# gio54321/quill-zkvm

Hardware: AMD Instinct MI355X
Metric: G1 MSM scalars/sec at 2^24 + sumcheck-prover ms at 2^20 vars (1/8 GPU) (higher is better)
Workload: dtype u256-montgomery (BN254 Fr scalars, Fq coordinates); 1 GPU; KZG commit / Pippenger G1 MSM, 2^24 BN254 scalars per GPU; parallelism=msm-shard-by-base-index x1

## Files before the change

### quill-zkvm_amd/csrc/msm.hip

```cpp
#include <stdlib.h>
#include <string.h>

#include "common.h"
#include "curve29.h"

using namespace qg;

namespace qg {

static constexpr int MSM_BLOCK = 256;

static int msm_window_bits(size_t n) {
  int best = 4;
  double best_cost = 1e300;
  for (int c = 4; c <= 22; c++) {
    const int W = (255 + c - 1) / c;
    const int k = 254 - c * (W - 1);
    if (k < 30 && (n >> k) > 4096) continue;
    const double cost = (double)n * W + 12.0 * (double)((size_t)1 << (c - 1));
    if (cost < best_cost) {
      best_cost = cost;
      best = c;
    }
  }
  return best;
}

QG_DEV Fr fr_canon29(const Fr& x) {
  F29<FrP> k = F29<FrP>::zero();
  k.l[0] = 32;
  return from29(canon29(mul29(to29(x), k)));
}

template <class Emit>
QG_DEV void for_each_digit(const Fr& canon, int c, int W, Emit&& emit) {
  uint32_t v[8];
#pragma unroll
  for (int i = 0; i < 8; i++) v[i] = canon.v[i];
  const uint32_t mask = (1u << c) - 1u;
  const uint32_t half = 1u << (c - 1);
  const uint32_t full = 1u << c;
  uint32_t carry = 0;
  for (int w = 0; w < W; w++) {
    const uint32_t d = (v[0] & mask) + carry;
    if (d > half) {
      carry = 1;
      const uint32_t mag = full - d;
      if (mag) emit(w, mag - 1, true);
    } else {
      carry = 0;
      if (d) emit(w, d - 1, false);
    }
#pragma unroll
    for (int i = 0; i < 7; i++) v[i] = __builtin_amdgcn_alignbit(v[i + 1], v[i], (uint32_t)c);
    v[7] >>= c;
  }
}

QG_DEV uint32_t xcd_tile(uint32_t b, uint32_t G) {
  const uint32_t x = b & 7u, q = G >> 3, r = G & 7u;
  return x * q + (x < r ? x : r) + (b >> 3);
}

static constexpr int SORT_BLOCK = 256;
static constexpr int SORT_TILE_MAX = 1024;
static constexpr size_t SORT_LDS_A = 72 * 1024;
static constexpr int SORT_CHUNK = 8192;
static constexpr int SORT_H_MAX = 1024, SORT_NL_MAX = 4096;

__global__ void k_handover_tag(uint32_t* hv, uint32_t w, uint32_t gen, uint32_t clear) {
  if (threadIdx.x == 0) {
    if (clear) hv[1] = hv[2] = hv[3] = 0u;
    hv[w] = gen;
  }
}

QG_DEV void msm_handover_check(uint32_t* hv, uint32_t w0, uint32_t nw, uint32_t gen, uint32_t bit) {
  if (hv == nullptr || threadIdx.x != 0) return;
  for (uint32_t w = w0; w < w0 + nw; w++)
    if (__hip_atomic_load(hv + w, __ATOMIC_RELAXED, __HIP_MEMORY_SCOPE_AGENT) != gen) {
      atomicOr(hv + 1, bit);
      return;
    }
}

__global__ void __launch_bounds__(SORT_BLOCK)
    k_sortA_hist(const Fr* __restrict__ scalars, size_t n, int c, int W, int LO, int H,
                 uint32_t nblk, uint32_t tile, uint32_t* __restrict__ hrow, Fr* __restrict__ canon,
                 uint32_t* hv, uint32_t gen, int wsel, int canon_ready) {
  extern __shared__ uint32_t hist[];
  msm_handover_check(hv, 0, 1, gen, 1u);
  for (int g = threadIdx.x; g < H; g += blockDim.x) hist[g] = 0;
  __syncthreads();
  const uint32_t tb = xcd_tile(blockIdx.x, nblk);
  const size_t base = (size_t)tb * tile;
  const size_t end = base + tile < n ? base + tile : n;
  for (size_t i = base + threadIdx.x; i < end; i += blockDim.x) {
    Fr s;
    if (canon_ready) {
      s = canon[i];
    } else {
      s = fr_canon29(scalars[i]);
      canon[i] = s;
    }
    for_each_digit(s, c, W, [&](int w, uint32_t b, bool) {
      if (wsel < 0 || w == wsel) atomicAdd(&hist[b >> LO], 1u);
    });
  }
  __syncthreads();
  for (int g = threadIdx.x; g < H; g += blockDim.x) hrow[(size_t)tb * H + g] = hist[g];
}

__global__ void __launch_bounds__(256)
    k_transpose32(const uint32_t* __restrict__ in, uint32_t rows, uint32_t cols,
                  uint32_t* __restrict__ out) {
  __shared__ uint32_t tile[32][33];
  const uint32_t c0 = blockIdx.x * 32, r0 = blockIdx.y * 32;
  const uint32_t tx = threadIdx.x & 31, ty = threadIdx.x >> 5;
  for (uint32_t k = ty; k < 32; k += 8)
    if (r0 + k < rows && c0 + tx < cols) tile[k][tx] = in[(size_t)(r0 + k) * cols + c0 + tx];
  __syncthreads();
  for (uint32_t k = ty; k < 32; k += 8)
    if (c0 + k < cols && r0 + tx < rows) out[(size_t)(c0 + k) * rows + r0 + tx] = tile[tx][k];
}

template <int BLK>
__device__ void lds_exscan(uint32_t* a, int n, uint32_t* tmp ) {
  const int per = (n + BLK - 1) / BLK;
  const int b = threadIdx.x * per;
  const int lane = threadIdx.x & 63, wid = threadIdx.x >> 6;
  uint32_t tot = 0;
  for (int k = 0; k < per; k++)
    if (b + k < n) tot += a[b + k];
  uint32_t inc = tot;
#pragma unroll
  for (int d = 1; d < 64; d <<= 1) {
    const uint32_t y = __shfl_up(inc, d, 64);
    if (lane >= d) inc += y;
  }
  if (lane == 63) tmp[wid] = inc;
  __syncthreads();
  uint32_t run = inc - tot;
  for (int w = 0; w < wid; w++) run += tmp[w];
  for (int k = 0; k < per; k++) {
    if (b + k < n) {
      const uint32_t v = a[b + k];
      a[b + k] = run;
      run += v;
    }
  }
  __syncthreads();
}

__device__ __forceinline__ int lds_upper(const uint32_t* off, int n, uint32_t p) {
  int lo = 0, hi = n;
  while (hi - lo > 1) {
    int mid = (lo + hi) >> 1;
    if (off[mid] <= p) lo = mid;
    else hi = mid;
  }
  return lo;
}

template <int BLK>
__global__ void __launch_bounds__(BLK)
    k_sortA_scatter(const Fr* __restrict__ canon, size_t n, size_t N, size_t off, int c, int W, int LO,
                    int H,
                    uint32_t nblk, uint32_t tile, const uint32_t* __restrict__ hrow,
                    const uint32_t* __restrict__ orow, uint32_t* __restrict__ tmp_e,
                    uint16_t* __restrict__ tmp_l, int wsel) {
  extern __shared__ __attribute__((aligned(16))) unsigned char smem[];
  uint32_t* ent = reinterpret_cast<uint32_t*>(smem);
  uint32_t* bkt = ent + (size_t)tile * (wsel < 0 ? W : 1);
  uint32_t* loff = bkt + (size_t)tile * (wsel < 0 ? W : 1);
  uint32_t* cur = loff + H;
  uint32_t* gb = cur + H;
  uint32_t* scr = gb + H;
  (void)scr;
  const uint32_t tb = xcd_tile(blockIdx.x, nblk);
  const size_t base = (size_t)tb * tile;
  const size_t end = base + tile < n ? base + tile : n;
  static_assert(SORT_TILE_MAX % BLK == 0, "pass-A tile must split evenly over the block");
  constexpr int PER = SORT_TILE_MAX / BLK;
  Fr sv[PER];
#pragma unroll
  for (int j = 0; j < PER; j++) {
    const size_t i = base + threadIdx.x + (size_t)j * BLK;
    if (i < end) sv[j] = canon[i];
  }
  for (int g = threadIdx.x; g < H; g += blockDim.x) {
    loff[g] = hrow[(size_t)tb * H + g];
    gb[g] = orow[(size_t)tb * H + g];
    cur[g] = 0;
  }
  __syncthreads();
#pragma unroll
  for (int j = 0; j < PER; j++) {
    const size_t i = base + threadIdx.x + (size_t)j * BLK;
    if (i >= end) break;
    for_each_digit(sv[j], c, W, [&](int w, uint32_t b, bool neg) {
      if (wsel >= 0 && w != wsel) return;
      const uint32_t g = b >> LO;
      const uint32_t slot = loff[g] + atomicAdd(&cur[g], 1u);
      const size_t row = (wsel < 0 ? (size_t)w * N : 0) + off + i;
      ent[slot] = (uint32_t)row | (neg ? 0x80000000u : 0u);
      bkt[slot] = b;
    });
  }
  __syncthreads();
  const uint32_t total = loff[H - 1] + cur[H - 1];
  const uint32_t lmask = (1u << LO) - 1u;
  for (uint32_t p = threadIdx.x; p < total; p += blockDim.x) {
    const uint32_t b = bkt[p];
    const uint32_t dst = gb[b >> LO] + p;
    tmp_e[dst] = ent[p];
    tmp_l[dst] = (uint16_t)(b & lmask);
  }
}

template <int BLK>
__global__ void __launch_bounds__(BLK)
    k_sortA_rows(uint32_t* __restrict__ hrow, uint32_t* __restrict__ orow, int H) {
  __shared__ uint32_t a[SORT_H_MAX], scr[BLK / 64];
  const size_t r = (size_t)blockIdx.x * H;
  for (int g = threadIdx.x; g < H; g += blockDim.x) a[g] = hrow[r + g];
  __syncthreads();
  lds_exscan<BLK>(a, H, scr);
  for (int g = threadIdx.x; g < H; g += blockDim.x) {
    hrow[r + g] = a[g];
    orow[r + g] -= a[g];
  }
}

__global__ void __launch_bounds__(1024)
    k_sort_chunks(const uint32_t* __restrict__ goff, uint32_t nblk, int H, uint32_t chunk,
                  uint32_t* __restrict__ gstart, uint32_t* __restrict__ cbase,
                  uint32_t* __restrict__ chunk_group, uint32_t* __restrict__ misc) {
  __shared__ uint32_t sh[1024];
  const int g = threadIdx.x;
  if (threadIdx.x >= 1 && threadIdx.x <= 3) misc[threadIdx.x] = threadIdx.x == 2 ? 0xffffffffu : 0u;
  const uint32_t total = goff[(size_t)H * nblk];
  uint32_t gs = 0, ge = 0, nch = 0;
  if (g < H) {
    gs = goff[(size_t)g * nblk];
    ge = (g + 1 < H) ? goff[(size_t)(g + 1) * nblk] : total;
    nch = (ge - gs + chunk - 1) / chunk;
    gstart[g] = gs;
  }
  sh[threadIdx.x] = nch;
  __syncthreads();
  for (int off = 1; off < 1024; off <<= 1) {
    uint32_t add = threadIdx.x >= (unsigned)off ? sh[threadIdx.x - off] : 0u;
    __syncthreads();
    sh[threadIdx.x] += add;
    __syncthreads();
  }
  const uint32_t cb = sh[threadIdx.x] - nch;
  if (g < H) {
    cbase[g] = cb;
    for (uint32_t k = 0; k < nch; k++) chunk_group[cb + k] = (uint32_t)g;
  }
  if (threadIdx.x == 1023) {
    gstart[H] = total;
    cbase[H] = sh[1023];
    misc[0] = sh[1023];
  }
}

template <int BLK, int CHUNK>
__global__ void __launch_bounds__(BLK)
    k_sortB_hist(const uint16_t* __restrict__ tmp_l, const uint32_t* __restrict__ gstart,
                 const uint32_t* __restrict__ cbase, const uint32_t* __restrict__ chunk_group,
                 const uint32_t* __restrict__ nchunks, int NL, uint32_t* __restrict__ chist) {
  extern __shared__ uint32_t hist[];
  const uint32_t nch = *nchunks;
  if (blockIdx.x >= nch) return;
  const uint32_t k = xcd_tile(blockIdx.x, nch);
  const uint32_t g = chunk_group[k];
  const uint32_t s = gstart[g] + (k - cbase[g]) * CHUNK;
  const uint32_t e = min(s + CHUNK, gstart[g + 1]);
  for (int l = threadIdx.x; l < NL; l += blockDim.x) hist[l] = 0;
  __syncthreads();
  constexpr int PER = CHUNK / BLK;
  uint32_t lv[PER];
#pragma unroll
  for (int j = 0; j < PER; j++) {
    const uint32_t p = s + threadIdx.x + j * BLK;
    lv[j] = p < e ? (uint32_t)tmp_l[p] : 0xffffffffu;
  }
#pragma unroll
  for (int j = 0; j < PER; j++)
    if (lv[j] != 0xffffffffu) atomicAdd(&hist[lv[j]], 1u);
  __syncthreads();
  for (int l = threadIdx.x; l < NL; l += blockDim.x) chist[(size_t)k * NL + l] = hist[l];
}

__global__ void k_sort_bucket_count(const uint32_t* __restrict__ cbase, const uint32_t* __restrict__ chist,
                                    int LO, uint32_t nb, uint32_t* __restrict__ counts) {
  const uint32_t b = blockIdx.x * blockDim.x + threadIdx.x;
  if (b >= nb) return;
  const uint32_t g = b >> LO, l = b & ((1u << LO) - 1);
  uint32_t c = 0;
#pragma unroll 8
  for (uint32_t k = cbase[g]; k < cbase[g + 1]; k++) c += chist[((size_t)k << LO) + l];
  counts[b] = c;
}

__global__ void k_sort_chunk_offsets(const uint32_t* __restrict__ cbase,
                                     const uint32_t* __restrict__ chist, int LO, uint32_t nb,
                                     const uint32_t* __restrict__ bstart,
                                     uint32_t* __restrict__ coff) {
  const uint32_t b = blockIdx.x * blockDim.x + threadIdx.x;
  if (b >= nb) return;
  const uint32_t g = b >> LO, l = b & ((1u << LO) - 1);
  uint32_t run = bstart[b];
#pragma unroll 8
  for (uint32_t k = cbase[g]; k < cbase[g + 1]; k++) {
    const size_t idx = ((size_t)k << LO) + l;
    coff[idx] = run;
    run += chist[idx];
  }
}

template <int BLK, int CHUNK>
__global__ void __launch_bounds__(BLK)
    k_sortB_scatter(const uint32_t* __restrict__ tmp_e, const uint16_t* __restrict__ tmp_l,
                    const uint32_t* __restrict__ gstart,
                    const uint32_t* __restrict__ cbase, const uint32_t* __restrict__ chunk_group,
                    const uint32_t* __restrict__ nchunks, int NL, const uint32_t* __restrict__ chist,
                    const uint32_t* __restrict__ coff, uint32_t* __restrict__ entries) {
  extern __shared__ __attribute__((aligned(16))) unsigned char smem[];
  uint32_t* e32 = reinterpret_cast<uint32_t*>(smem);
  static_assert(CHUNK % BLK == 0, "pass-B chunk must split evenly over the block");
  uint16_t* bins = reinterpret_cast<uint16_t*>(e32 + CHUNK);
  uint32_t* loff = reinterpret_cast<uint32_t*>(bins + CHUNK);
  uint32_t* cur = loff + NL;
  uint32_t* cb = cur + NL;
  uint32_t* scr = cb + NL;
  const uint32_t nch = *nchunks;
  if (blockIdx.x >= nch) return;
  const uint32_t k = xcd_tile(blockIdx.x, nch);
  const uint32_t g = chunk_group[k];
  const uint32_t s = gstart[g] + (k - cbase[g]) * CHUNK;
  const uint32_t e = min(s + CHUNK, gstart[g + 1]);
  constexpr int PER = CHUNK / BLK;
  uint32_t ev[PER], lv[PER];
#pragma unroll
  for (int j = 0; j < PER; j++) {
    const uint32_t p = s + threadIdx.x + j * BLK;
    lv[j] = p < e ? (uint32_t)tmp_l[p] : 0xffffffffu;
    ev[j] = p < e ? tmp_e[p] : 0u;
  }
  for (int l = threadIdx.x; l < NL; l += blockDim.x) {
    loff[l] = chist[(size_t)k * NL + l];
    cur[l] = 0;
  }
  __syncthreads();
  lds_exscan<BLK>(loff, NL, scr);
  for (int l = threadIdx.x; l < NL; l += blockDim.x) cb[l] = coff[(size_t)k * NL + l] - loff[l];
#pragma unroll
  for (int j = 0; j < PER; j++) {
    if (lv[j] == 0xffffffffu) continue;
    const uint32_t l = lv[j];
    const uint32_t slot = loff[l] + atomicAdd(&cur[l], 1u);
    e32[slot] = ev[j];
    bins[slot] = (uint16_t)l;
  }
  __syncthreads();
  for (uint32_t q = threadIdx.x; q < e - s; q += blockDim.x) entries[cb[bins[q]] + q] = e32[q];
}

__global__ void k_scan32_tiles(const uint32_t* __restrict__ in, size_t n, uint32_t* __restrict__ out,
                               uint32_t* __restrict__ tile_tot) {
  __shared__ uint32_t sh[256];
  const size_t base = ((size_t)blockIdx.x * 256 + threadIdx.x) * 8;
  uint32_t v[8], tot = 0;
  for (int k = 0; k < 8; k++) {
    v[k] = base + k < n ? in[base + k] : 0u;
    tot += v[k];
  }
  sh[threadIdx.x] = tot;
  __syncthreads();
  for (int off = 1; off < 256; off <<= 1) {
    uint32_t add = threadIdx.x >= (unsigned)off ? sh[threadIdx.x - off] : 0u;
    __syncthreads();
    sh[threadIdx.x] += add;
    __syncthreads();
  }
  uint32_t run = sh[threadIdx.x] - tot;
  for (int k = 0; k < 8; k++) {
    if (base + k < n) out[base + k] = run;
    run += v[k];
  }
  if (threadIdx.x == 255) tile_tot[blockIdx.x] = sh[255];
}

__global__ void __launch_bounds__(1024)
    k_scan32_top(uint32_t* __restrict__ tile_tot, int ntiles, uint32_t* __restrict__ out_total) {
  __shared__ uint32_t sh[1024];
  const int per = (ntiles + 1023) / 1024;
  const int base = threadIdx.x * per;
  uint32_t tot = 0;
  for (int k = 0; k < per; k++)
    if (base + k < ntiles) tot += tile_tot[base + k];
  sh[threadIdx.x] = tot;
  __syncthreads();
  for (int off = 1; off < 1024; off <<= 1) {
    uint32_t add = threadIdx.x >= (unsigned)off ? sh[threadIdx.x - off] : 0u;
    __syncthreads();
    sh[threadIdx.x] += add;
    __syncthreads();
  }
  uint32_t run = sh[threadIdx.x] - tot;
  for (int k = 0; k < per; k++) {
    if (base + k < ntiles) {
      uint32_t t = tile_tot[base + k];
      tile_tot[base + k] = run;
      run += t;
    }
  }
  if (threadIdx.x == 1023) *out_total = sh[1023];
}

__global__ void k_scan32_add(const uint32_t* __restrict__ tile_off, size_t n, uint32_t* __restrict__ out) {
  const size_t i = (size_t)blockIdx.x * blockDim.x + threadIdx.x;
  if (i < n) out[i] += tile_off[i / 2048];
}

static constexpr int SCAN_PER_THREAD = 8;
static constexpr int SCAN_BLOCK = 256;
static constexpr int SCAN_TILE = SCAN_PER_THREAD * SCAN_BLOCK;

__device__ __forceinline__ uint2 scan_val(const uint32_t* counts, size_t i, size_t nb, uint32_t L) {
  uint32_t c = i < nb ? counts[i] : 0u;
  return make_uint2(c, (c + L - 1) / L);
}

__global__ void k_scan_tiles(const uint32_t* __restrict__ counts, size_t nb, uint32_t L,
                             uint32_t* __restrict__ bstart, uint2* __restrict__ tile_tot,
                             uint32_t* __restrict__ max_tpb) {
  __shared__ uint2 sh[SCAN_BLOCK];
  size_t base = (size_t)blockIdx.x * SCAN_TILE + threadIdx.x * SCAN_PER_THREAD;
  uint2 v[SCAN_PER_THREAD];
  uint2 tot = make_uint2(0, 0);
  uint32_t mx = 0;
  for (int k = 0; k < SCAN_PER_THREAD; k++) {
    v[k] = scan_val(counts, base + k, nb, L);
    tot.x += v[k].x;
    tot.y += v[k].y;
    mx = max(mx, v[k].y);
  }
  if (mx > 1) atomicMax(max_tpb, mx);
// ... 628 lines not shown
  int idx = blockIdx.x * blockDim.x + threadIdx.x;
  if (idx >= 32 * 256) return;
  int k = idx >> 8, j = idx & 255;
  G1Xyzz acc = xyzz_mul_small(bases[k], (uint32_t)j);
  fb[idx] = xyzz_to_affine(acc);
}

__global__ void k_fb_mul(const G1Affine* __restrict__ fb, const Fr* __restrict__ scal, size_t n,
                         G1Affine* __restrict__ out) {
  size_t i = (size_t)blockIdx.x * blockDim.x + threadIdx.x;
  if (i >= n) return;
  Fr s = from_mont(scal[i]);
  G1Xyzz acc = G1Xyzz::infinity();
  for (int k = 0; k < 32; k++) {
    uint32_t byte = (s.v[k >> 2] >> (8 * (k & 3))) & 255u;
    if (byte) acc = xyzz_add_affine(acc, fb[k * 256 + byte]);
  }
  out[i] = xyzz_to_affine(acc);
}

__global__ void k_import_bases(const uint64_t* __restrict__ xy, const uint8_t* __restrict__ inf,
                               size_t n, G1Affine* __restrict__ out) {
  size_t i = (size_t)blockIdx.x * blockDim.x + threadIdx.x;
  if (i >= n) return;
  G1Affine a;
  for (int l = 0; l < 4; l++) {
    uint64_t x = xy[8 * i + l], y = xy[8 * i + 4 + l];
    a.x.v[2 * l] = (uint32_t)x;
    a.x.v[2 * l + 1] = (uint32_t)(x >> 32);
    a.y.v[2 * l] = (uint32_t)y;
    a.y.v[2 * l + 1] = (uint32_t)(y >> 32);
  }
  if (inf && inf[i]) a = G1Affine::infinity();
  out[i] = a;
}

static void srs_build_tables(qg_ctx* ctx, qg_srs* srs, const G1Affine* base) {
  QgTimed tm(ctx, "srs_shift");
  hipLaunchKernelGGL(k_srs_pack, dim3(div_up(srs->n, 256)), dim3(256), 0, ctx->stream, base,
                     srs->n, srs->d_table);
  QG_LAUNCH_CHECK();
  for (int w = 1; w < srs->tables; w++) {
    hipLaunchKernelGGL(k_srs_shift, dim3(div_up(srs->n, 256)), dim3(256), 0, ctx->stream,
                       srs->d_table, srs->n, w, srs->c);
    QG_LAUNCH_CHECK();
  }
}

static qg_srs* srs_alloc(qg_ctx* ctx, size_t n, bool oneshot = false) {
  qg_srs* srs = new qg_srs();
  srs->ctx = ctx;
  srs->n = n;
  int ct = msm_window_bits(n);
  if (oneshot) ct = std::min(ct, 18);
  if (const char* ov = getenv("QG_MSM_WINDOW_BITS")) ct = atoi(ov);
  QG_CHECK(ct >= 4 && ct <= 26, QG_ERR_INVALID, "MSM window bits out of range");
  srs->W = (255 + ct - 1) / ct;
  srs->c = (255 + srs->W - 1) / srs->W;
  srs->tables = oneshot ? 1 : srs->W;
  hipError_t e = hipMalloc(&srs->d_table, (size_t)srs->tables * n * sizeof(MsmPt));
  if (e != hipSuccess) {
    delete srs;
    throw Error(QG_ERR_OOM, "qg_srs: hipMalloc of the window tables failed");
  }
  return srs;
}

struct MsmRun {
  bool empty = true;
  uint32_t L = 1, T = 4;
  size_t nslots = 0;
  X29Raw* partial = nullptr;
  uint32_t* owner = nullptr;
  uint32_t* bstart = nullptr;
  uint32_t* misc = nullptr;
  const uint32_t* h_mx = nullptr;
  hipEvent_t ev_mx = nullptr;
  uint32_t gen = 0;
};
static constexpr int MSM_MAX_BATCH = 1024;

struct SortGeom {
  uint32_t blkA, tile, blkB, chunk;
};

static constexpr size_t SORT_WIDE_MIN = (size_t)1 << 26;
static constexpr size_t SORT_MID_MIN = (size_t)1 << 20;
static SortGeom sort_geometry(size_t max_entries, int WE, bool narrow) {
  SortGeom g;
  const bool wide = !narrow && max_entries >= SORT_WIDE_MIN;
  const bool mid = !narrow && max_entries >= SORT_MID_MIN;
  g.blkA = wide ? 1024 : mid ? 512 : SORT_BLOCK;
  g.blkB = wide ? 1024 : mid ? 512 : SORT_BLOCK;
  g.chunk = wide ? 16384 : SORT_CHUNK;
  while (g.blkA > (uint32_t)SORT_BLOCK &&
         (size_t)g.blkA * WE * 8 + (3 * (size_t)SORT_H_MAX + 16) * 4 > 160 * 1024)
    g.blkA >>= 1;
  if (const char* ov = getenv("QG_SORT_BLOCK_A")) g.blkA = (uint32_t)atoi(ov);
  if (const char* ov = getenv("QG_SORT_BLOCK_B")) g.blkB = (uint32_t)atoi(ov);
  if (const char* ov = getenv("QG_SORT_CHUNK")) g.chunk = (uint32_t)atoi(ov);
  g.tile = SORT_TILE_MAX;
  while (g.tile > 64 && (size_t)g.tile * WE * 8 > SORT_LDS_A) g.tile >>= 1;
  if (g.blkA > SORT_BLOCK && g.blkA <= (uint32_t)SORT_TILE_MAX) g.tile = std::max(g.tile, g.blkA);
  if (const char* ov = getenv("QG_SORT_TILE")) g.tile = (uint32_t)atoi(ov);
  QG_CHECK(g.tile >= 64 && g.tile <= (uint32_t)SORT_TILE_MAX && (g.tile & (g.tile - 1)) == 0,
           QG_ERR_INVALID, "QG_SORT_TILE must be a power of two in [64, 1024]");
  QG_CHECK(g.blkA == 256 || ((g.blkA == 512 || g.blkA == 1024) && g.tile >= g.blkA),
           QG_ERR_INVALID, "no pass-A sort kernel for this QG_SORT_BLOCK_A / QG_SORT_TILE");
  QG_CHECK((g.blkB == 256 && g.chunk == 8192) || (g.blkB == 512 && g.chunk == 8192) ||
               (g.blkB == 512 && g.chunk == 16384) || (g.blkB == 1024 && g.chunk == 16384),
           QG_ERR_INVALID, "no pass-B sort kernel for this QG_SORT_BLOCK_B / QG_SORT_CHUNK");
  return g;
}

static void sort_lds_attr(qg_ctx* ctx, const void* fn, const std::string& key) {
  if (ctx->memo.count(key)) return;
  QG_HIP(hipFuncSetAttribute(fn, hipFuncAttributeMaxDynamicSharedMemorySize, 160 * 1024));
  ctx->memo[key] = "1";
}

#define QG_SORT_DISPATCH_A(blk, F) \
  do {                             \
    if ((blk) == 256) { F(256); }  \
    else if ((blk) == 512) { F(512); } \
    else { F(1024); }              \
  } while (0)
#define QG_SORT_DISPATCH_B(blk, chunk, F)                   \
  do {                                                      \
    if ((blk) == 256) { F(256, 8192); }                     \
    else if ((blk) == 512 && (chunk) == 8192) { F(512, 8192); } \
    else if ((blk) == 512) { F(512, 16384); }               \
    else { F(1024, 16384); }                                \
  } while (0)

static MsmRun msm_accumulate_phase(qg_ctx* ctx, const qg_srs* srs, const Fr* d_scalars, size_t n,
                                   int slot, size_t srs_off = 0, hipStream_t bst = nullptr,
                                   bool reserve = false, uint32_t* hv = nullptr, uint32_t hgen = 0,
                                   int wsel = -1, bool canon_ready = false) {
  QG_CHECK(srs_off <= srs->n && n <= srs->n - srs_off, QG_ERR_INVALID, "MSM length exceeds the SRS");
  MsmRun run;
  const std::string sfx = "#" + std::to_string(slot);
  const bool side = bst != nullptr && bst != ctx->stream;
  if (!bst) bst = ctx->stream;
  const std::string tg = side ? "@" + std::to_string(slot & 1) : std::string();
  if (n > 0) {
    const int c = srs->c, W = srs->W;
    QG_CHECK((wsel < 0) == (srs->tables == W) && wsel < W, QG_ERR_INVALID,
             "MSM window selection does not match the SRS tables");
    const int WE = wsel < 0 ? W : 1;
    const uint32_t nb = 1u << (c - 1);
    const size_t max_entries = n * (size_t)WE;
    QG_CHECK((size_t)W * srs->n < 0x80000000ull, QG_ERR_UNSUPPORTED, "SRS table index overflow");
    QG_CHECK(max_entries < 0xffffffffull, QG_ERR_UNSUPPORTED, "too many MSM entries");
    const int BB = c - 1, LO = (BB + 1) / 2, HI = BB - LO;
    const int H = 1 << HI, NL = 1 << LO;
    const SortGeom geo = sort_geometry(max_entries, WE, side || wsel >= 0);
    const uint32_t tile = geo.tile, chunk = geo.chunk;
    const uint32_t nblk = div_up(n, tile);
    const size_t nghist = (size_t)H * nblk;
    const size_t max_chunks = max_entries / chunk + H + 1;
    uint32_t* ghist = ctx->scratch_as<uint32_t>("msm_ghist" + tg, nghist + 1);
    uint32_t* goff = ctx->scratch_as<uint32_t>("msm_goff" + tg, nghist + 1);
    uint32_t* gtiles = ctx->scratch_as<uint32_t>("msm_gtiles" + tg, div_up(nghist, 2048) + 1);
    uint32_t* gstart = ctx->scratch_as<uint32_t>("msm_gstart" + tg, H + 1);
    uint32_t* cbase = ctx->scratch_as<uint32_t>("msm_cbase" + tg, H + 1);
    uint32_t* cgroup = ctx->scratch_as<uint32_t>("msm_cgroup" + tg, max_chunks);
    uint32_t* misc = ctx->scratch_as<uint32_t>("msm_misc" + sfx, 5);
    uint32_t* chist = ctx->scratch_as<uint32_t>("msm_chist" + tg, max_chunks * NL);
    uint32_t* coff = ctx->scratch_as<uint32_t>("msm_coff" + tg, max_chunks * NL);
    uint32_t* tmp_e = ctx->scratch_as<uint32_t>("msm_tmp_e" + tg, max_entries + 1);
    uint16_t* tmp_l = ctx->scratch_as<uint16_t>("msm_tmp_l" + tg, max_entries + 1);
    uint32_t* hrow = ctx->scratch_as<uint32_t>("msm_hrow" + tg, nghist + 1);
    uint32_t* orow = ctx->scratch_as<uint32_t>("msm_orow" + tg, nghist + 1);
    Fr* canon = ctx->scratch_as<Fr>("msm_canon" + tg, n);
    uint32_t* counts = ctx->scratch_as<uint32_t>("msm_counts" + tg, nb);
    uint32_t* bstart = ctx->scratch_as<uint32_t>("msm_bstart" + sfx, nb + 1);
    uint32_t* entries = ctx->scratch_as<uint32_t>("msm_entries" + tg, max_entries + 1);
    if (reserve) return run;
    const int ntiles = (int)div_up(nb, SCAN_TILE);
    uint2* tile_tot = ctx->scratch_as<uint2>("msm_tiles" + tg, ntiles);
    uint32_t L;
    if (const char* ov = getenv("QG_MSM_ROUNDS")) {
      const int rounds = atoi(ov);
      QG_CHECK(rounds >= 1 && rounds <= 64, QG_ERR_INVALID, "QG_MSM_ROUNDS out of range");
      const size_t resident = (size_t)ctx->num_cus() * 16 * 64;
      L = 4;
      while ((size_t)L * resident * rounds < max_entries) L <<= 1;
    } else {
      int elog = max_entries >= ((size_t)1 << 27) ? 7 : 6;
      while (elog > 2 && (max_entries >> elog) < (size_t)ctx->num_cus() * 16 * 64 * 3) elog--;
      int emin = 0;
      size_t cpb = side ? 2 : 4;
      if (const char* ov = getenv("QG_MSM_CPB")) cpb = (size_t)std::max(1, atoi(ov));
      while (emin < 7 && ((size_t)1 << emin) * cpb * nb < max_entries) emin++;
      elog = std::max(elog, emin);
      L = 1u << elog;
    }
    if (const char* ov = getenv("QG_MSM_ELOG")) L = 1u << atoi(ov);
    bool pf = max_entries >= ((size_t)1 << 27);
    if (const char* ov = getenv("QG_MSM_PF")) pf = atoi(ov) != 0;
    bool coop = max_entries >= ((size_t)1 << 25);
    if (const char* ov = getenv("QG_MSM_COOP")) coop = atoi(ov) != 0;
    int eqk = side ? 1 : 0;
    if (const char* ov = getenv("QG_MSM_EQSPLIT")) eqk = atoi(ov);
    {
      const int k = eqk;
      if (k > 0) {
        const size_t wpe = coop ? QG_COOP_WPE : (pf ? 3 : 4);
        const size_t resident = (size_t)ctx->num_cus() * 4 * wpe * 64;
        const size_t lq = (div_up(max_entries, resident * (size_t)k) + 3) & ~(size_t)3;
        L = (uint32_t)std::max<size_t>(4, lq);
      }
    }
    const uint32_t T = std::max<uint32_t>(4, (uint32_t)div_up(div_up(max_entries, nb), L) + 2);
    QG_CHECK(L >= 4 && L <= 65536 && (L & 3u) == 0, QG_ERR_INVALID, "MSM chunk length out of range");
    const uint64_t Lm = ~0ull / L + 1;
    const size_t max_threads = div_up(max_entries, L);
    const size_t nslots = max_threads + nb + 1;
    X29Raw* partial = ctx->scratch_as<X29Raw>("msm_partial" + sfx, nslots);
    uint32_t* owner = ctx->scratch_as<uint32_t>("msm_owner" + sfx, nslots);
    QG_CHECK(ntiles <= 1024 * 64 && H <= SORT_H_MAX && NL <= SORT_NL_MAX, QG_ERR_UNSUPPORTED,
             "bucket count too large");
    const size_t smemA = (size_t)tile * WE * 8 + (3 * (size_t)H + geo.blkA / 64) * 4;
    const size_t smemB = (size_t)chunk * 6 + (3 * (size_t)NL + geo.blkB / 64) * 4;
    QG_CHECK(smemA <= 160 * 1024 && smemB <= 160 * 1024, QG_ERR_UNSUPPORTED,
             "sort tile / chunk exceeds LDS");
    QG_CHECK(nslots < 0xffffffffull && max_chunks < 0xffffffffull, QG_ERR_UNSUPPORTED,
             "MSM too large");

    {
      QgTimed tm(ctx, side ? "msm_bucketing_side" : "msm_bucketing", bst);
      hipLaunchKernelGGL(k_sortA_hist, dim3(nblk), dim3(SORT_BLOCK), H * sizeof(uint32_t),
                         bst, d_scalars, n, c, W, LO, H, nblk, tile, hrow, canon, hv, hgen, wsel,
                         canon_ready ? 1 : 0);
      QG_LAUNCH_CHECK();
      hipLaunchKernelGGL(k_transpose32, dim3(div_up(H, 32), div_up(nblk, 32)), dim3(256), 0,
                         bst, hrow, nblk, (uint32_t)H, ghist);
      QG_LAUNCH_CHECK();
      const unsigned gt = div_up(nghist, 2048);
      QG_CHECK(gt <= 1024u * 1024u, QG_ERR_UNSUPPORTED, "histogram too large");
      hipLaunchKernelGGL(k_scan32_tiles, dim3(gt), dim3(256), 0, bst, ghist, nghist, goff,
                         gtiles);
      QG_LAUNCH_CHECK();
      hipLaunchKernelGGL(k_scan32_top, dim3(1), dim3(1024), 0, bst, gtiles, (int)gt,
                         goff + nghist);
      QG_LAUNCH_CHECK();
      hipLaunchKernelGGL(k_scan32_add, dim3(div_up(nghist, 256)), dim3(256), 0, bst, gtiles,
                         nghist, goff);
      QG_LAUNCH_CHECK();
      hipLaunchKernelGGL(k_transpose32, dim3(div_up(nblk, 32), div_up(H, 32)), dim3(256), 0,
                         bst, goff, (uint32_t)H, nblk, orow);
      QG_LAUNCH_CHECK();
#define QG_SORT_A_LAUNCH(BLK)                                                                    \
  hipLaunchKernelGGL(k_sortA_rows<BLK>, dim3(nblk), dim3(BLK), 0, bst, hrow, orow, H);           \
  QG_LAUNCH_CHECK();                                                                             \
  sort_lds_attr(ctx, reinterpret_cast<const void*>(&k_sortA_scatter<BLK>), "msm_lds_attrA" #BLK); \
  hipLaunchKernelGGL(k_sortA_scatter<BLK>, dim3(nblk), dim3(BLK), smemA, bst, canon, n, srs->n,  \
                     srs_off, c, W, LO, H, nblk, tile, hrow, orow, tmp_e, tmp_l, wsel);          \
  QG_LAUNCH_CHECK()
      QG_SORT_DISPATCH_A(geo.blkA, QG_SORT_A_LAUNCH);
#undef QG_SORT_A_LAUNCH
      hipLaunchKernelGGL(k_sort_chunks, dim3(1), dim3(1024), 0, bst, goff, nblk, H, chunk,
                         gstart, cbase, cgroup, misc);
      QG_LAUNCH_CHECK();
#define QG_SORT_B_HIST(BLK, CHUNK)                                                              \
  hipLaunchKernelGGL(HIP_KERNEL_NAME(k_sortB_hist<BLK, CHUNK>), dim3((unsigned)max_chunks),     \
                     dim3(BLK), NL * sizeof(uint32_t), bst, tmp_l, gstart, cbase, cgroup, misc, \
                     NL, chist);                                                                \
  QG_LAUNCH_CHECK()
      QG_SORT_DISPATCH_B(geo.blkB, chunk, QG_SORT_B_HIST);
#undef QG_SORT_B_HIST
      hipLaunchKernelGGL(k_sort_bucket_count, dim3(div_up(nb, 256)), dim3(256), 0, bst,
                         cbase, chist, LO, nb, counts);
      QG_LAUNCH_CHECK();
      hipLaunchKernelGGL(k_scan_tiles, dim3(ntiles), dim3(SCAN_BLOCK), 0, bst, counts,
                         (size_t)nb, L, bstart, tile_tot, misc + 1);
      QG_LAUNCH_CHECK();
      hipLaunchKernelGGL(k_scan_top, dim3(1), dim3(1024), 0, bst, tile_tot, ntiles,
                         bstart, (size_t)nb);
      QG_LAUNCH_CHECK();
      run.gen = ++ctx->msm_gen;
      hipLaunchKernelGGL(k_scan_add, dim3(div_up(nb, 256)), dim3(256), 0, bst, tile_tot,
                         (size_t)nb, bstart, counts, L, T, misc, run.gen, owner, nslots);
      QG_LAUNCH_CHECK();
      {
        QG_CHECK(slot >= 0 && slot < MSM_MAX_BATCH, QG_ERR_UNSUPPORTED, "MSM batch too large");
        uint32_t* hmx =
            reinterpret_cast<uint32_t*>(ctx->pinned_get("msm_mx", MSM_MAX_BATCH * 4 * sizeof(uint32_t)));
        QG_HIP(hipMemcpyAsync(hmx + 4 * slot, misc + 1, 4 * sizeof(uint32_t), hipMemcpyDeviceToHost,
                              bst));
        run.ev_mx = ctx->ev_get();
        QG_HIP(hipEventRecord(run.ev_mx, bst));
        run.h_mx = hmx + 4 * slot;
      }
      hipLaunchKernelGGL(k_sort_chunk_offsets, dim3(div_up(nb, 256)), dim3(256), 0, bst,
                         cbase, chist, LO, nb, bstart, coff);
      QG_LAUNCH_CHECK();
#define QG_SORT_B_SCATTER(BLK, CHUNK)                                                          \
  sort_lds_attr(ctx, reinterpret_cast<const void*>(&k_sortB_scatter<BLK, CHUNK>),              \
                "msm_lds_attrB" #BLK "_" #CHUNK);                                              \
  hipLaunchKernelGGL(HIP_KERNEL_NAME(k_sortB_scatter<BLK, CHUNK>), dim3((unsigned)max_chunks), \
                     dim3(BLK), smemB, bst, tmp_e, tmp_l, gstart, cbase, cgroup, misc, NL,     \
                     chist, coff, entries);                                                    \
  QG_LAUNCH_CHECK()
      QG_SORT_DISPATCH_B(geo.blkB, chunk, QG_SORT_B_SCATTER);
#undef QG_SORT_B_SCATTER
    }
    const hipStream_t ast = bst;
    {
      QgTimed tm(ctx, "msm_accumulate", ast);
      if (coop)
        hipLaunchKernelGGL(k_msm_accumulate_coop, dim3(div_up(max_threads, MSM_BLOCK)),
                           dim3(MSM_BLOCK), 0, ast, srs->d_table, entries, bstart, nb, L, Lm,
                           partial, owner);
      else if (pf)
        hipLaunchKernelGGL(k_msm_accumulate<true>, dim3(div_up(max_threads, MSM_BLOCK)),
                           dim3(MSM_BLOCK), 0, ast, srs->d_table, entries, bstart, nb, L, Lm,
                           partial, owner);
      else
        hipLaunchKernelGGL(k_msm_accumulate<false>, dim3(div_up(max_threads, MSM_BLOCK)),
                           dim3(MSM_BLOCK), 0, ast, srs->d_table, entries, bstart, nb, L, Lm,
                           partial, owner);
      QG_LAUNCH_CHECK();
    }
    run.empty = n == 0;
    run.L = L;
    run.T = T;
    run.nslots = nslots;
    run.partial = partial;
    run.owner = owner;
    run.bstart = bstart;
    run.misc = misc;
  }
  return run;
}

static void msm_reduce_phase(qg_ctx* ctx, const qg_srs* srs, const std::vector<MsmRun>& runs,
                             std::vector<G1Xyzz>& out, uint32_t* hv = nullptr, uint32_t hgen = 0,
                             uint32_t* h_err = nullptr) {
  const uint32_t k = (uint32_t)runs.size();
  out.assign(k, G1Xyzz::infinity());
  std::vector<uint32_t> live;
  for (uint32_t i = 0; i < k; i++)
    if (!runs[i].empty) live.push_back(i);
  if (live.empty()) {
    if (hv) {
      QG_HIP(hipMemcpyAsync(h_err, hv + 1, sizeof(uint32_t), hipMemcpyDeviceToHost, ctx->stream));
      ctx->sync();
    }
    return;
  }
  QG_CHECK(live.size() <= (size_t)MSM_MAX_BATCH, QG_ERR_UNSUPPORTED, "MSM batch too large");
  const uint32_t kl = (uint32_t)live.size();
  const uint32_t nb = 1u << (srs->c - 1);
  std::vector<uint32_t> mx(3 * (size_t)kl);
  if (const char* ov = getenv("QG_MSM_SYNC_PLAN"))
    if (atoi(ov) != 0) QG_HIP(hipStreamSynchronize(ctx->stream));
  for (uint32_t q = 0; q < kl; q++) {
    const MsmRun& r = runs[live[q]];
    QG_CHECK(r.ev_mx && r.h_mx, QG_ERR_ASSERT, "MSM run without its bucket-scan event");
    QG_HIP(hipEventSynchronize(r.ev_mx));
    if (r.h_mx[3] == r.gen) {
      for (int i = 0; i < 3; i++) mx[3 * q + i] = r.h_mx[i];
    } else {
      QG_HIP(hipStreamSynchronize(ctx->stream));
      uint32_t w[4];
      QG_HIP(hipMemcpy(w, r.misc + 1, sizeof(w), hipMemcpyDeviceToHost));
      QG_CHECK(w[3] == r.gen, QG_ERR_ASSERT, "MSM bucket-scan plan words of another run");
      for (int i = 0; i < 3; i++) mx[3 * q + i] = w[i];
      ctx->msm_plan_refetch++;
    }
  }
  for (const MsmRun& r : runs)
    if (r.ev_mx) ctx->event_pool.push_back(r.ev_mx);
  const size_t lanes = (size_t)ctx->num_cus() * 4 * 64;
  int slog1 = 0;
  while (slog1 < 12 && ((size_t)kl * nb >> (slog1 + 1)) >= lanes) slog1++;
  if (const char* ov = getenv("QG_MSM_SLOG1")) slog1 = atoi(ov);
  QG_CHECK(slog1 >= 0 && slog1 <= 12, QG_ERR_INVALID, "QG_MSM_SLOG1 out of range");
  int gl1 = 4;
  if (const char* ov = getenv("QG_MSM_GL1")) gl1 = atoi(ov);
  QG_CHECK(gl1 >= 0 && gl1 <= 6, QG_ERR_INVALID, "QG_MSM_GL1 out of range");
  const uint32_t g1 = div_up(div_up(nb, (size_t)1 << slog1), MSM_BLOCK);
  const uint32_t m1 = g1 * (MSM_BLOCK >> gl1);
  const uint32_t m2 = div_up(m1, 16);
  G1Xyzz* A1 = ctx->scratch_as<G1Xyzz>("msm_redA1", (size_t)kl * m1);
// ... 742 lines not shown
```

Baseline: 964.4 million scalars/s.

## Make MSM sort scatter kernels persistent with double-buffered prefetch of next tile

Both sort-scatter passes (A: digit decomposition into groups, B: chunk-local bucket scatter) become persistent grid-stride kernels. In the wide configuration each block loads the next tile's scalars or entries and its histogram and offset rows into registers and a second LDS row buffer while it processes the current tile, so global-memory latency is hidden. The LDS atomic slot claims are also batched ILP=4 at a time, to overlap LDS atomic latency. The cost is extra LDS and registers per block, lower occupancy, and an occupancy-based grid size with environment overrides.

```diff
diff --git a/quill-zkvm_amd/csrc/msm.hip b/quill-zkvm_amd/csrc/msm.hip
--- a/quill-zkvm_amd/csrc/msm.hip
+++ b/quill-zkvm_amd/csrc/msm.hip
@@ -57,6 +57,22 @@
   }
 }
 
+struct DigitStep {
+  uint32_t b;
+  bool neg, any;
+};
+QG_DEV DigitStep digit_step(uint32_t (&v)[8], uint32_t& carry, int c) {
+  const uint32_t full = 1u << c;
+  const uint32_t d = (v[0] & (full - 1u)) + carry;
+  const bool neg = d > (full >> 1);
+  const uint32_t mag = neg ? full - d : d;
+  carry = neg ? 1u : 0u;
+#pragma unroll
+  for (int i = 0; i < 7; i++) v[i] = __builtin_amdgcn_alignbit(v[i + 1], v[i], (uint32_t)c);
+  v[7] >>= c;
+  return DigitStep{mag - 1u, neg, mag != 0u};
+}
+
 QG_DEV uint32_t xcd_tile(uint32_t b, uint32_t G) {
   const uint32_t x = b & 7u, q = G >> 3, r = G & 7u;
   return x * q + (x < r ? x : r) + (b >> 3);
@@ -67,6 +83,7 @@
 static constexpr size_t SORT_LDS_A = 72 * 1024;
 static constexpr int SORT_CHUNK = 8192;
 static constexpr int SORT_H_MAX = 1024, SORT_NL_MAX = 4096;
+static constexpr int SORT_ILP = 4;
 
 __global__ void k_handover_tag(uint32_t* hv, uint32_t w, uint32_t gen, uint32_t clear) {
   if (threadIdx.x == 0) {
@@ -162,59 +179,142 @@
   return lo;
 }
 
-template <int BLK>
+static constexpr int QG_WAIT_VM0 = 0x0F70;
+
+template <int BLK, bool PF>
 __global__ void __launch_bounds__(BLK)
     k_sortA_scatter(const Fr* __restrict__ canon, size_t n, size_t N, size_t off, int c, int W, int LO,
                     int H,
                     uint32_t nblk, uint32_t tile, const uint32_t* __restrict__ hrow,
                     const uint32_t* __restrict__ orow, uint32_t* __restrict__ tmp_e,
-                    uint16_t* __restrict__ tmp_l, int wsel) {
+                    uint16_t* __restrict__ tmp_l, int wsel, uint32_t rstride) {
   extern __shared__ __attribute__((aligned(16))) unsigned char smem[];
   uint32_t* ent = reinterpret_cast<uint32_t*>(smem);
   uint32_t* bkt = ent + (size_t)tile * (wsel < 0 ? W : 1);
-  uint32_t* loff = bkt + (size_t)tile * (wsel < 0 ? W : 1);
-  uint32_t* cur = loff + H;
-  uint32_t* gb = cur + H;
-  uint32_t* scr = gb + H;
-  (void)scr;
-  const uint32_t tb = xcd_tile(blockIdx.x, nblk);
-  const size_t base = (size_t)tb * tile;
-  const size_t end = base + tile < n ? base + tile : n;
+  uint32_t* rows = bkt + (size_t)tile * (wsel < 0 ? W : 1);
+  uint32_t k = blockIdx.x;
+  if (k >= nblk) return;
   static_assert(SORT_TILE_MAX % BLK == 0, "pass-A tile must split evenly over the block");
-  constexpr int PER = SORT_TILE_MAX / BLK;
+  static_assert(SORT_H_MAX % BLK == 0, "pass-A rows must split evenly over the block");
+  constexpr int PER = SORT_TILE_MAX / BLK, RPT = SORT_H_MAX / BLK, ILP = SORT_ILP;
+  auto load_scalars = [&](uint32_t tb, Fr* s) {
+    const size_t base = (size_t)tb * tile;
+    const size_t end = base + tile < n ? base + tile : n;
+#pragma unroll
+    for (int j = 0; j < PER; j++) {
+      const size_t i = base + threadIdx.x + (size_t)j * BLK;
+      if (i < end) s[j] = canon[i];
+    }
+  };
+  auto load = [&](uint32_t kk, Fr* s, uint32_t* h, uint32_t* o) {
+    const uint32_t tb = xcd_tile(kk, nblk);
+    load_scalars(tb, s);
+#pragma unroll
+    for (int r = 0; r < RPT; r++) {
+      const int g = threadIdx.x + r * BLK;
+      if (g < H) {
+        h[r] = hrow[(size_t)tb * H + g];
+        o[r] = orow[(size_t)tb * H + g];
+      }
+    }
+  };
+  auto put_rows = [&](uint32_t* loff, const uint32_t* h, const uint32_t* o) {
+#pragma unroll
+    for (int r = 0; r < RPT; r++) {
+      const int g = threadIdx.x + r * BLK;
+      if (g < H) {
+        loff[g] = h[r];
+        loff[H + g] = 0;
+        loff[2 * H + g] = o[r];
+      }
+    }
+  };
   Fr sv[PER];
-#pragma unroll
-  for (int j = 0; j < PER; j++) {
-    const size_t i = base + threadIdx.x + (size_t)j * BLK;
-    if (i < end) sv[j] = canon[i];
-  }
-  for (int g = threadIdx.x; g < H; g += blockDim.x) {
-    loff[g] = hrow[(size_t)tb * H + g];
-    gb[g] = orow[(size_t)tb * H + g];
-    cur[g] = 0;
-  }
-  __syncthreads();
-#pragma unroll
-  for (int j = 0; j < PER; j++) {
-    const size_t i = base + threadIdx.x + (size_t)j * BLK;
-    if (i >= end) break;
-    for_each_digit(sv[j], c, W, [&](int w, uint32_t b, bool neg) {
-      if (wsel >= 0 && w != wsel) return;
-      const uint32_t g = b >> LO;
-      const uint32_t slot = loff[g] + atomicAdd(&cur[g], 1u);
-      const size_t row = (wsel < 0 ? (size_t)w * N : 0) + off + i;
-      ent[slot] = (uint32_t)row | (neg ? 0x80000000u : 0u);
-      bkt[slot] = b;
-    });
-  }
-  __syncthreads();
-  const uint32_t total = loff[H - 1] + cur[H - 1];
-  const uint32_t lmask = (1u << LO) - 1u;
-  for (uint32_t p = threadIdx.x; p < total; p += blockDim.x) {
-    const uint32_t b = bkt[p];
-    const uint32_t dst = gb[b >> LO] + p;
-    tmp_e[dst] = ent[p];
-    tmp_l[dst] = (uint16_t)(b & lmask);
+  uint32_t hr[RPT], gr[RPT];
+  uint32_t* loff = rows;
+  if (PF) {
+    load(k, sv, hr, gr);
+    put_rows(loff, hr, gr);
+    __builtin_amdgcn_s_waitcnt(QG_WAIT_VM0);
+    __syncthreads();
+  }
+  for (;;) {
+    const uint32_t kn = k + gridDim.x;
+    const bool more = kn < nblk;
+    Fr nsv[PER];
+    uint32_t nhr[RPT], ngr[RPT];
+    if (PF) {
+      if (more) load(kn, nsv, nhr, ngr);
+    } else {
+      const uint32_t tb = xcd_tile(k, nblk);
+      load_scalars(tb, sv);
+      for (int g = threadIdx.x; g < H; g += blockDim.x) {
+        loff[g] = hrow[(size_t)tb * H + g];
+        loff[2 * H + g] = orow[(size_t)tb * H + g];
+        loff[H + g] = 0;
+      }
+      __syncthreads();
+    }
+    uint32_t* cur = loff + H;
+    const uint32_t* gb = cur + H;
+    const size_t base = (size_t)xcd_tile(k, nblk) * tile;
+    const size_t end = base + tile < n ? base + tile : n;
+#pragma unroll
+    for (int j = 0; j < PER; j++) {
+      const size_t i = base + threadIdx.x + (size_t)j * BLK;
+      if (i >= end) break;
+      uint32_t v[8], carry = 0;
+#pragma unroll
+      for (int q = 0; q < 8; q++) v[q] = sv[j].v[q];
+      for (int w0 = 0; w0 < W; w0 += ILP) {
+        uint32_t r[ILP], lo[ILP], g[ILP], en[ILP], bb[ILP];
+        bool ok[ILP];
+#pragma unroll
+        for (int q = 0; q < ILP; q++) {
+          const int w = w0 + q;
+          const DigitStep t = digit_step(v, carry, c);
+          ok[q] = w < W && t.any && (wsel < 0 || w == wsel);
+          const size_t row = (wsel < 0 ? (size_t)w * N : 0) + off + i;
+          en[q] = (uint32_t)row | (t.neg ? 0x80000000u : 0u);
+          bb[q] = t.b;
+          g[q] = t.b >> LO;
+          r[q] = lo[q] = 0;
+          if (ok[q]) {
+            lo[q] = loff[g[q]];
+            r[q] = atomicAdd(&cur[g[q]], 1u);
+          }
+        }
+#pragma unroll
+        for (int q = 0; q < ILP; q++) {
+          if (!ok[q]) continue;
+          const uint32_t slot = lo[q] + r[q];
+          ent[slot] = en[q];
+          bkt[slot] = bb[q];
+        }
+      }
+    }
+    uint32_t* nloff = loff == rows ? rows + rstride : rows;
+    if (PF) {
+      __builtin_amdgcn_s_waitcnt(QG_WAIT_VM0);
+      if (more) put_rows(nloff, nhr, ngr);
+    }
+    __syncthreads();
+    const uint32_t total = loff[H - 1] + cur[H - 1];
+    const uint32_t lmask = (1u << LO) - 1u;
+    for (uint32_t p = threadIdx.x; p < total; p += blockDim.x) {
+      const uint32_t b = bkt[p];
+      const uint32_t dst = gb[b >> LO] + p;
+      tmp_e[dst] = ent[p];
+      tmp_l[dst] = (uint16_t)(b & lmask);
+    }
+    if (!more) break;
+    __syncthreads();
+    k = kn;
+    if (PF) {
+#pragma unroll
+      for (int j = 0; j < PER; j++) sv[j] = nsv[j];
+      loff = nloff;
+    }
   }
 }
 
@@ -322,52 +422,147 @@
   }
 }
 
-template <int BLK, int CHUNK>
+template <int BLK, int CHUNK, bool PF>
 __global__ void __launch_bounds__(BLK)
     k_sortB_scatter(const uint32_t* __restrict__ tmp_e, const uint16_t* __restrict__ tmp_l,
                     const uint32_t* __restrict__ gstart,
                     const uint32_t* __restrict__ cbase, const uint32_t* __restrict__ chunk_group,
                     const uint32_t* __restrict__ nchunks, int NL, const uint32_t* __restrict__ chist,
-                    const uint32_t* __restrict__ coff, uint32_t* __restrict__ entries) {
+                    const uint32_t* __restrict__ coff, uint32_t* __restrict__ entries,
+                    uint32_t rstride) {
   extern __shared__ __attribute__((aligned(16))) unsigned char smem[];
   uint32_t* e32 = reinterpret_cast<uint32_t*>(smem);
   static_assert(CHUNK % BLK == 0, "pass-B chunk must split evenly over the block");
+  static_assert(SORT_NL_MAX % BLK == 0, "pass-B rows must split evenly over the block");
   uint16_t* bins = reinterpret_cast<uint16_t*>(e32 + CHUNK);
-  uint32_t* loff = reinterpret_cast<uint32_t*>(bins + CHUNK);
-  uint32_t* cur = loff + NL;
-  uint32_t* cb = cur + NL;
-  uint32_t* scr = cb + NL;
+  uint32_t* scr = reinterpret_cast<uint32_t*>(bins + CHUNK);
+  uint32_t* rows = scr + BLK / 64;
   const uint32_t nch = *nchunks;
-  if (blockIdx.x >= nch) return;
-  const uint32_t k = xcd_tile(blockIdx.x, nch);
-  const uint32_t g = chunk_group[k];
-  const uint32_t s = gstart[g] + (k - cbase[g]) * CHUNK;
-  const uint32_t e = min(s + CHUNK, gstart[g + 1]);
-  constexpr int PER = CHUNK / BLK;
-  uint32_t ev[PER], lv[PER];
-#pragma unroll
-  for (int j = 0; j < PER; j++) {
-    const uint32_t p = s + threadIdx.x + j * BLK;
-    lv[j] = p < e ? (uint32_t)tmp_l[p] : 0xffffffffu;
-    ev[j] = p < e ? tmp_e[p] : 0u;
-  }
-  for (int l = threadIdx.x; l < NL; l += blockDim.x) {
-    loff[l] = chist[(size_t)k * NL + l];
-    cur[l] = 0;
-  }
-  __syncthreads();
-  lds_exscan<BLK>(loff, NL, scr);
-  for (int l = threadIdx.x; l < NL; l += blockDim.x) cb[l] = coff[(size_t)k * NL + l] - loff[l];
-#pragma unroll
-  for (int j = 0; j < PER; j++) {
-    if (lv[j] == 0xffffffffu) continue;
-    const uint32_t l = lv[j];
-    const uint32_t slot = loff[l] + atomicAdd(&cur[l], 1u);
-    e32[slot] = ev[j];
-    bins[slot] = (uint16_t)l;
-  }
-  __syncthreads();
-  for (uint32_t q = threadIdx.x; q < e - s; q += blockDim.x) entries[cb[bins[q]] + q] = e32[q];
+  uint32_t k = blockIdx.x;
+  if (k >= nch) return;
+  constexpr int PER = CHUNK / BLK, RPT = SORT_NL_MAX / BLK, ILP = SORT_ILP;
+  auto span = [&](uint32_t kk, uint32_t& ck, uint32_t& s, uint32_t& e) {
+    ck = xcd_tile(kk, nch);
+    const uint32_t g = chunk_group[ck];
+    s = gstart[g] + (ck - cbase[g]) * CHUNK;
+    e = min(s + CHUNK, gstart[g + 1]);
+  };
+  auto load_entries = [&](uint32_t s, uint32_t e, uint32_t* ev, uint32_t* lv) {
+#pragma unroll
+    for (int j = 0; j < PER; j++) {
+      const uint32_t p = s + threadIdx.x + j * BLK;
+      lv[j] = p < e ? (uint32_t)tmp_l[p] : 0xffffffffu;
+      ev[j] = p < e ? tmp_e[p] : 0u;
+    }
+  };
+  auto load = [&](uint32_t ck, uint32_t s, uint32_t e, uint32_t* ev, uint32_t* lv, uint32_t* h,
+                  uint32_t* o) {
+    load_entries(s, e, ev, lv);
+#pragma unroll
+    for (int r = 0; r < RPT; r++) {
+      const int l = threadIdx.x + r * BLK;
+      if (l < NL) {
+        h[r] = chist[(size_t)ck * NL + l];
+        o[r] = coff[(size_t)ck * NL + l];
+      }
+    }
+  };
+  auto put_rows = [&](uint32_t* loff, const uint32_t* h) {
+#pragma unroll
+    for (int r = 0; r < RPT; r++) {
+      const int l = threadIdx.x + r * BLK;
+      if (l < NL) {
+        loff[l] = h[r];
+        loff[NL + l] = 0;
+      }
+    }
+  };
+  uint32_t ck = 0, s = 0, e = 0, nck = 0, ns = 0, ne = 0;
+  uint32_t ev[PER], lv[PER], hr[RPT], co[RPT];
+  uint32_t* loff = rows;
+  if (PF) {
+    span(k, ck, s, e);
+    if (k + gridDim.x < nch) span(k + gridDim.x, nck, ns, ne);
+    load(ck, s, e, ev, lv, hr, co);
+    put_rows(loff, hr);
+    __builtin_amdgcn_s_waitcnt(QG_WAIT_VM0);
+    __syncthreads();
+  }
+  for (;;) {
+    const uint32_t kn = k + gridDim.x;
+    const bool more = kn < nch;
+    uint32_t nev[PER], nlv[PER], nhr[RPT], nco[RPT];
+    uint32_t fck = 0, fs = 0, fe = 0;
+    if (PF) {
+      if (more) {
+        load(nck, ns, ne, nev, nlv, nhr, nco);
+        if (kn + gridDim.x < nch) span(kn + gridDim.x, fck, fs, fe);
+      }
+    } else {
+      span(k, ck, s, e);
+      load_entries(s, e, ev, lv);
+      for (int l = threadIdx.x; l < NL; l += blockDim.x) {
+        loff[l] = chist[(size_t)ck * NL + l];
+        loff[NL + l] = 0;
+      }
+      __syncthreads();
+    }
+    uint32_t* cur = loff + NL;
+    uint32_t* cb = cur + NL;
+    lds_exscan<BLK>(loff, NL, scr);
+    if (PF) {
+#pragma unroll
+      for (int r = 0; r < RPT; r++) {
+        const int l = threadIdx.x + r * BLK;
+        if (l < NL) cb[l] = co[r] - loff[l];
+      }
+    } else {
+      for (int l = threadIdx.x; l < NL; l += blockDim.x) cb[l] = coff[(size_t)ck * NL + l] - loff[l];
+    }
+    static_assert(PER % ILP == 0, "pass-B entries per thread must split into ILP groups");
+#pragma unroll
+    for (int j0 = 0; j0 < PER; j0 += ILP) {
+      uint32_t r[ILP], lo[ILP];
+#pragma unroll
+      for (int q = 0; q < ILP; q++) {
+        r[q] = lo[q] = 0;
+        if (lv[j0 + q] != 0xffffffffu) {
+          lo[q] = loff[lv[j0 + q]];
+          r[q] = atomicAdd(&cur[lv[j0 + q]], 1u);
+        }
+      }
+#pragma unroll
+      for (int q = 0; q < ILP; q++) {
+        if (lv[j0 + q] == 0xffffffffu) continue;
+        const uint32_t l = lv[j0 + q];
+        const uint32_t slot = lo[q] + r[q];
+        e32[slot] = ev[j0 + q];
+        bins[slot] = (uint16_t)l;
+      }
+    }
+    uint32_t* nloff = loff == rows ? rows + rstride : rows;
+    if (PF) {
+      __builtin_amdgcn_s_waitcnt(QG_WAIT_VM0);
+      if (more) put_rows(nloff, nhr);
+    }
+    __syncthreads();
+    for (uint32_t q = threadIdx.x; q < e - s; q += blockDim.x) entries[cb[bins[q]] + q] = e32[q];
+    if (!more) break;
+    __syncthreads();
+    k = kn;
+    if (PF) {
+#pragma unroll
+      for (int j = 0; j < PER; j++) {
+        ev[j] = nev[j];
+        lv[j] = nlv[j];
+      }
+#pragma unroll
+      for (int r = 0; r < RPT; r++) co[r] = nco[r];
+      loff = nloff;
+      s = ns, e = ne;
+      nck = fck, ns = fs, ne = fe;
+    }
+  }
 }
 
 __global__ void k_scan32_tiles(const uint32_t* __restrict__ in, size_t n, uint32_t* __restrict__ out,
@@ -1162,10 +1357,20 @@
 
 struct SortGeom {
   uint32_t blkA, tile, blkB, chunk;
+  int gridA, gridB;
+  bool wide;
 };
 
 static constexpr size_t SORT_WIDE_MIN = (size_t)1 << 26;
 static constexpr size_t SORT_MID_MIN = (size_t)1 << 20;
+static constexpr int SORT_GRID_MAX = 1 << 20;
+static int sort_grid_override(const char* ov) {
+  char* end = nullptr;
+  const long v = strtol(ov, &end, 10);
+  QG_CHECK(end != ov && *end == 0 && v >= 0 && v <= SORT_GRID_MAX, QG_ERR_INVALID,
+           "QG_SORT_GRID_A / QG_SORT_GRID_B must be a block count in [0, 2^20]");
+  return (int)v;
+}
 static SortGeom sort_geometry(size_t max_entries, int WE, bool narrow) {
   SortGeom g;
   const bool wide = !narrow && max_entries >= SORT_WIDE_MIN;
@@ -1173,12 +1378,16 @@
   g.blkA = wide ? 1024 : mid ? 512 : SORT_BLOCK;
   g.blkB = wide ? 1024 : mid ? 512 : SORT_BLOCK;
   g.chunk = wide ? 16384 : SORT_CHUNK;
+  g.wide = wide;
+  g.gridA = g.gridB = -1;
   while (g.blkA > (uint32_t)SORT_BLOCK &&
          (size_t)g.blkA * WE * 8 + (3 * (size_t)SORT_H_MAX + 16) * 4 > 160 * 1024)
     g.blkA >>= 1;
   if (const char* ov = getenv("QG_SORT_BLOCK_A")) g.blkA = (uint32_t)atoi(ov);
   if (const char* ov = getenv("QG_SORT_BLOCK_B")) g.blkB = (uint32_t)atoi(ov);
   if (const char* ov = getenv("QG_SORT_CHUNK")) g.chunk = (uint32_t)atoi(ov);
+  if (const char* ov = getenv("QG_SORT_GRID_A")) g.gridA = sort_grid_override(ov);
+  if (const char* ov = getenv("QG_SORT_GRID_B")) g.gridB = sort_grid_override(ov);
   g.tile = SORT_TILE_MAX;
   while (g.tile > 64 && (size_t)g.tile * WE * 8 > SORT_LDS_A) g.tile >>= 1;
   if (g.blkA > SORT_BLOCK && g.blkA <= (uint32_t)SORT_TILE_MAX) g.tile = std::max(g.tile, g.blkA);
@@ -1197,6 +1406,25 @@
   if (ctx->memo.count(key)) return;
   QG_HIP(hipFuncSetAttribute(fn, hipFuncAttributeMaxDynamicSharedMemorySize, 160 * 1024));
   ctx->memo[key] = "1";
+}
+
+static constexpr size_t SORT_GRID_ROUNDS = 8;
+static uint32_t sort_scatter_grid(qg_ctx* ctx, const void* fn, const std::string& key, int blk,
+                                  size_t smem, int forced, bool multi, size_t count) {
+  if (forced > 0) return (uint32_t)forced;
+  if (forced == 0 || !multi) return (uint32_t)count;
+  const std::string mk = key + "_occ" + std::to_string(smem);
+  auto it = ctx->memo.find(mk);
+  int occ = 0;
+  if (it == ctx->memo.end()) {
+    QG_HIP(hipOccupancyMaxActiveBlocksPerMultiprocessor(&occ, fn, blk, smem));
+    ctx->memo[mk] = std::to_string(occ);
+  } else {
+    occ = std::stoi(it->second);
+  }
+  QG_CHECK(occ >= 1, QG_ERR_DEVICE, "sort scatter kernel cannot be resident");
+  const size_t blocks = (((size_t)occ * ctx->num_cus()) & ~(size_t)7) * SORT_GRID_ROUNDS;
+  return (uint32_t)(blocks >= 8 && blocks < count ? blocks : count);
 }
 
 #define QG_SORT_DISPATCH_A(blk, F) \
@@ -1301,10 +1529,24 @@
     uint32_t* owner = ctx->scratch_as<uint32_t>("msm_owner" + sfx, nslots);
     QG_CHECK(ntiles <= 1024 * 64 && H <= SORT_H_MAX && NL <= SORT_NL_MAX, QG_ERR_UNSUPPORTED,
              "bucket count too large");
-    const size_t smemA = (size_t)tile * WE * 8 + (3 * (size_t)H + geo.blkA / 64) * 4;
-    const size_t smemB = (size_t)chunk * 6 + (3 * (size_t)NL + geo.blkB / 64) * 4;
+    size_t smemA = (size_t)tile * WE * 8 + (3 * (size_t)H + geo.blkA / 64) * 4;
+    size_t smemB = (size_t)chunk * 6 + (3 * (size_t)NL + geo.blkB / 64) * 4;
     QG_CHECK(smemA <= 160 * 1024 && smemB <= 160 * 1024, QG_ERR_UNSUPPORTED,
              "sort tile / chunk exceeds LDS");
+    const void* fnA = reinterpret_cast<const void*>(&k_sortA_scatter<1024, true>);
+    const void* fnB = reinterpret_cast<const void*>(&k_sortB_scatter<1024, 16384, true>);
+    const size_t smemA2 = smemA + 3 * (size_t)H * 4, smemB2 = smemB + 3 * (size_t)NL * 4;
+    const bool canA = geo.blkA == 1024 && smemA2 <= 160 * 1024;
+    const bool canB = geo.blkB == 1024 && smemB2 <= 160 * 1024;
+    if (canA) sort_lds_attr(ctx, fnA, "msm_lds_attrA1024pf");
+    if (canB) sort_lds_attr(ctx, fnB, "msm_lds_attrB1024_16384pf");
+    const uint32_t gridA = sort_scatter_grid(ctx, fnA, "msm_sortA1024pf", 1024, smemA2, geo.gridA,
+                                             geo.wide && canA, nblk);
+    const uint32_t gridB = sort_scatter_grid(ctx, fnB, "msm_sortB1024pf", 1024, smemB2, geo.gridB,
+                                             geo.wide && canB, max_chunks);
+    const bool pfA = canA && gridA < nblk, pfB = canB && gridB < max_chunks;
+    if (pfA) smemA = smemA2;
+    if (pfB) smemB = smemB2;
     QG_CHECK(nslots < 0xffffffffull && max_chunks < 0xffffffffull, QG_ERR_UNSUPPORTED,
              "MSM too large");
 
@@ -1334,9 +1576,17 @@
 #define QG_SORT_A_LAUNCH(BLK)                                                                    \
   hipLaunchKernelGGL(k_sortA_rows<BLK>, dim3(nblk), dim3(BLK), 0, bst, hrow, orow, H);           \
   QG_LAUNCH_CHECK();                                                                             \
-  sort_lds_attr(ctx, reinterpret_cast<const void*>(&k_sortA_scatter<BLK>), "msm_lds_attrA" #BLK); \
-  hipLaunchKernelGGL(k_sortA_scatter<BLK>, dim3(nblk), dim3(BLK), smemA, bst, canon, n, srs->n,  \
-                     srs_off, c, W, LO, H, nblk, tile, hrow, orow, tmp_e, tmp_l, wsel);          \
+  if (pfA) {                                                                                     \
+    hipLaunchKernelGGL(HIP_KERNEL_NAME(k_sortA_scatter<1024, true>), dim3(gridA), dim3(1024),    \
+                       smemA, bst, canon, n, srs->n, srs_off, c, W, LO, H, nblk, tile, hrow,     \
+                       orow, tmp_e, tmp_l, wsel, 3u * (uint32_t)H);                              \
+  } else {                                                                                       \
+    sort_lds_attr(ctx, reinterpret_cast<const void*>(&k_sortA_scatter<BLK, false>),              \
+                  "msm_lds_attrA" #BLK);                                                         \
+    hipLaunchKernelGGL(HIP_KERNEL_NAME(k_sortA_scatter<BLK, false>), dim3(gridA), dim3(BLK),     \
+                       smemA, bst, canon, n, srs->n, srs_off, c, W, LO, H, nblk, tile, hrow,     \
+                       orow, tmp_e, tmp_l, wsel, 0u);                                            \
+  }                                                                                              \
   QG_LAUNCH_CHECK()
       QG_SORT_DISPATCH_A(geo.blkA, QG_SORT_A_LAUNCH);
 #undef QG_SORT_A_LAUNCH
@@ -1377,11 +1627,17 @@
                          cbase, chist, LO, nb, bstart, coff);
       QG_LAUNCH_CHECK();
 #define QG_SORT_B_SCATTER(BLK, CHUNK)                                                          \
-  sort_lds_attr(ctx, reinterpret_cast<const void*>(&k_sortB_scatter<BLK, CHUNK>),              \
-                "msm_lds_attrB" #BLK "_" #CHUNK);                                              \
-  hipLaunchKernelGGL(HIP_KERNEL_NAME(k_sortB_scatter<BLK, CHUNK>), dim3((unsigned)max_chunks), \
-                     dim3(BLK), smemB, bst, tmp_e, tmp_l, gstart, cbase, cgroup, misc, NL,     \
-                     chist, coff, entries);                                                    \
+  if (pfB) {                                                                                   \
+    hipLaunchKernelGGL(HIP_KERNEL_NAME(k_sortB_scatter<1024, 16384, true>), dim3(gridB),       \
+                       dim3(1024), smemB, bst, tmp_e, tmp_l, gstart, cbase, cgroup, misc, NL,  \
+                       chist, coff, entries, 3u * (uint32_t)NL);                               \
+  } else {                                                                                     \
+    sort_lds_attr(ctx, reinterpret_cast<const void*>(&k_sortB_scatter<BLK, CHUNK, false>),     \
+                  "msm_lds_attrB" #BLK "_" #CHUNK);                                            \
+    hipLaunchKernelGGL(HIP_KERNEL_NAME(k_sortB_scatter<BLK, CHUNK, false>), dim3(gridB),       \
+                       dim3(BLK), smemB, bst, tmp_e, tmp_l, gstart, cbase, cgroup, misc, NL,   \
+                       chist, coff, entries, 0u);                                              \
+  }                                                                                            \
   QG_LAUNCH_CHECK()
       QG_SORT_DISPATCH_B(geo.blkB, chunk, QG_SORT_B_SCATTER);
 #undef QG_SORT_B_SCATTER
```

Result: faster. 981.0 million scalars/s, median of 6 (+1.7%).
